# anibali/dsnt-pose2d

Measured on AMD Instinct MI355X. Metric: images/sec (train step, 256x256, 16 joints), higher is better.
Workload: dtype f32; 1 GPU; hg2 + DSNT + JS reg, 256x256 -> 64x64x16, batch 32 per GPU, RMSprop lr 2.5e-4, train step fwd+loss+bwd+optim; global_batch=32, parallelism=dp1, launches_fwd=210

## Files before the change

### dsnt-pose2d_amd/csrc/api.cpp

```cpp
#include "common.h"
#include <string.h>

static thread_local char g_err[512] = "";

int dsnt_set_error(int code, const char* fmt, ...) {
    va_list ap;
    va_start(ap, fmt);
    vsnprintf(g_err, sizeof(g_err), fmt, ap);
    va_end(ap);
    return code;
}

int dsnt_device_id(void) {
    int d = 0;
    if (hipGetDevice(&d) != hipSuccess || d < 0) d = 0;
    return d < DSNT_MAX_DEVICES ? d : DSNT_MAX_DEVICES - 1;
}

int dsnt_device_cus(void) {
    static std::atomic<int> cus[DSNT_MAX_DEVICES];
    const int d = dsnt_device_id();
    int c = cus[d].load(std::memory_order_acquire);
    if (!c) {
        hipDeviceProp_t prop;
        int dev = 0;
        c = (hipGetDevice(&dev) == hipSuccess && hipGetDeviceProperties(&prop, dev) == hipSuccess && prop.multiProcessorCount > 0)
                ? prop.multiProcessorCount : 256;
        cus[d].store(c, std::memory_order_release);
    }
    return c;
}

extern "C" int dsnt_version(void) { return 132; }
extern "C" const char* dsnt_last_error(void) { return g_err; }

#include <vector>
#include <new>

struct dsnt_list {
    struct Entry {
        int kind;
        int lane, src, dst;
        mutable hipEvent_t ev;
        std::function<void(hipStream_t)> fn;
    };
    std::vector<Entry> entries;
    std::vector<size_t> seg_start;
    dsnt_list() { seg_start.push_back(0); }
// ... 78 lines not shown
```

### dsnt-pose2d_amd/csrc/bn.hip

```cpp
#include "common.h"
#include <string.h>
#include "bn_pro.h"
#include "ew_bodies.h"

template <int MODE>
__global__ __launch_bounds__(256) void tile_reduce_kernel(
    const float* __restrict__ a, const float* __restrict__ x, const float* __restrict__ scale,
    const float* __restrict__ shift, const float* __restrict__ mean,
    const float* __restrict__ invstd, int relu, float* __restrict__ partial, long M, int C, int cgs,
    const float* __restrict__ ymask = nullptr, float* __restrict__ dz_out = nullptr) {
    __shared__ float red[256 * 8];
    const int tid = threadIdx.x;
    const int C4 = C >> 2;
    const int rpar = 256 / cgs;
    const int cg_l = tid % cgs, rl = tid / cgs;
    const bool active = rl < rpar;
    const long row0 = (long)blockIdx.x * TILE_ROWS;
    const long row1 = row0 + TILE_ROWS < M ? row0 + TILE_ROWS : M;
    for (int cg0 = blockIdx.y * cgs; cg0 < C4; cg0 += cgs * gridDim.y) {
        const int cg = cg0 + cg_l;
        float4 s1 = make_float4(0.f, 0.f, 0.f, 0.f), s2 = s1;
        if (active && cg < C4) {
            float4 sc, sh, mu, is;
            if (MODE == 1) {
// ... 326 lines not shown
                                long n4) {
    for (long i = (long)blockIdx.x * blockDim.x + threadIdx.x; i < n4; i += (long)gridDim.x * blockDim.x) {
        const float4 g = dy[i], v = y[i];
        dz[i] = make_float4(v.x > 0.f ? g.x : 0.f, v.y > 0.f ? g.y : 0.f, v.z > 0.f ? g.z : 0.f, v.w > 0.f ? g.w : 0.f);
    }
}

extern "C" int dsnt_relu_bwd(const float* dy, const float* y, float* dz, int64_t n, void* stream) {
    DSNT_REQUIRE(dy && y && dz && n > 0 && n % 4 == 0, DSNT_ERR_ARG, "dsnt_relu_bwd: bad argument");
    DSNT_REQUIRE(dsnt_aligned16(dy) && dsnt_aligned16(y) && dsnt_aligned16(dz), DSNT_ERR_ALIGN, "dsnt_relu_bwd: alignment");
    DSNT_LAUNCH(relu_bwd_kernel, dim3(flat_grid(n / 4, 256)), dim3(256), 0, (hipStream_t)stream,
                       (const float4*)dy, (const float4*)y, (float4*)dz, (long)(n / 4));
    DSNT_CHECK_LAUNCH("dsnt_relu_bwd");
}

struct BnApplyVec { float4 sc, sh, mu, is, c0, c1; };
__device__ __forceinline__ float4 bn_apply_one(const float4 g, const float4 xv, const BnApplyVec& v, int relu) {
    float4 dz = g;
    if (relu) {
        if (fmaf(xv.x, v.sc.x, v.sh.x) <= 0.f) dz.x = 0.f;
        if (fmaf(xv.y, v.sc.y, v.sh.y) <= 0.f) dz.y = 0.f;
        if (fmaf(xv.z, v.sc.z, v.sh.z) <= 0.f) dz.z = 0.f;
        if (fmaf(xv.w, v.sc.w, v.sh.w) <= 0.f) dz.w = 0.f;
    }
    float4 o;
    o.x = v.sc.x * (dz.x - v.c0.x - (xv.x - v.mu.x) * v.is.x * v.c1.x);
    o.y = v.sc.y * (dz.y - v.c0.y - (xv.y - v.mu.y) * v.is.y * v.c1.y);
    o.z = v.sc.z * (dz.z - v.c0.z - (xv.z - v.mu.z) * v.is.z * v.c1.z);
    o.w = v.sc.w * (dz.w - v.c0.w - (xv.w - v.mu.w) * v.is.w * v.c1.w);
    return o;
}
struct BnApplyP {
    const float4* da; const float4* x; const float4* scale; const float4* shift; const float4* mean; const float4* invstd;
    const float4* coef; int relu; float4* dx; const float4* base; long n4; int C4; unsigned* amax; BnBwdProP pro;
};
template <bool FIXED>
__global__ void bn_act_bwd_apply_kernel(BnApplyP q) {
    __shared__ double pro_sh[512];
    const float4* __restrict__ da = q.da; const float4* __restrict__ x = q.x; const float4* __restrict__ scale = q.scale;
    const float4* __restrict__ shift = q.shift; const float4* __restrict__ mean = q.mean; const float4* __restrict__ invstd = q.invstd;
    const float4* coef = q.coef; const int relu = q.relu; float4* dx = q.dx; const float4* base = q.base;
    const long n4 = q.n4; const int C4 = q.C4; unsigned* __restrict__ amax = q.amax; const BnBwdProP pro = q.pro;
    const bool accumulate = base != nullptr;
    const int wg = blockIdx.x, nwg = gridDim.x;
    if (pro.partial) {
        bn_pro_backward<256>(pro, pro_sh, wg == 0);
        __syncthreads();
    }
    float am = 0.f;
    const long stride = (long)nwg * 256;
    long i = threadIdx.x < 256 ? (long)wg * 256 + threadIdx.x : n4;
    auto vec = [&](int cg) {
        BnApplyVec v;
        v.sc = scale[cg]; v.sh = shift[cg]; v.mu = mean[cg]; v.is = invstd[cg]; v.c0 = coef[cg]; v.c1 = coef[C4 + cg];
        return v;
    };
    auto amx = [&](const float4 o) { am = fmaxf(fmaxf(fmaxf(fabsf(o.x), fabsf(o.y)), fmaxf(fabsf(o.z), fabsf(o.w))), am); };
    if (FIXED) {
        const BnApplyVec v = vec((int)((i < n4 ? i : 0) % C4));
        for (; i + stride < n4; i += 2 * stride) {
            const float4 g0 = da[i], x0 = x[i], g1 = da[i + stride], x1 = x[i + stride];
            float4 p0 = make_float4(0.f, 0.f, 0.f, 0.f), p1 = p0;
            if (accumulate) { p0 = base[i]; p1 = base[i + stride]; }
            float4 o0 = bn_apply_one(g0, x0, v, relu), o1 = bn_apply_one(g1, x1, v, relu);
            if (accumulate) {
                o0.x += p0.x; o0.y += p0.y; o0.z += p0.z; o0.w += p0.w;
                o1.x += p1.x; o1.y += p1.y; o1.z += p1.z; o1.w += p1.w;
            }
            dx[i] = o0; dx[i + stride] = o1;
            amx(o0); amx(o1);
        }
        if (i < n4) {
            float4 o = bn_apply_one(da[i], x[i], v, relu);
            if (accumulate) { const float4 p = base[i]; o.x += p.x; o.y += p.y; o.z += p.z; o.w += p.w; }
            dx[i] = o;
            amx(o);
        }
    } else {
        for (; i < n4; i += stride) {
            float4 o = bn_apply_one(da[i], x[i], vec((int)(i % C4)), relu);
            if (accumulate) { const float4 p = base[i]; o.x += p.x; o.y += p.y; o.z += p.z; o.w += p.w; }
            dx[i] = o;
            amx(o);
        }
    }
    if (amax) amax_commit(am, amax);
}

static int bn_act_bwd_apply_impl(const float* da, const float* x, const float* scale, const float* shift,
                                 const float* mean, const float* invstd, const float* coef, int relu, float* dx,
                                 int accumulate, int64_t M, int C, float* amax, void* stream, const BnBwdProP* pro, const float* base) {
    DSNT_REQUIRE(da && x && scale && shift && mean && invstd && coef && dx && M > 0 && C > 0,
                 DSNT_ERR_ARG, "dsnt_bn_act_bwd_apply: bad argument");
    DSNT_REQUIRE(C % 4 == 0 && dsnt_aligned16(da) && dsnt_aligned16(x) && dsnt_aligned16(dx) &&
                 dsnt_aligned16(coef) && dsnt_aligned16(base), DSNT_ERR_ALIGN, "dsnt_bn_act_bwd_apply: alignment");
    if (!base && accumulate) base = dx;
    const long n4 = (long)M * C / 4;
    int grid = flat_grid(n4, 256);
    BnBwdProP q;
    memset(&q, 0, sizeof(q));
    if (pro) {
        q = *pro;
        if (grid > 128) grid = 128;
    }
    const BnApplyP ap{(const float4*)da, (const float4*)x, (const float4*)scale, (const float4*)shift, (const float4*)mean,
                      (const float4*)invstd, (const float4*)coef, relu, (float4*)dx, (const float4*)base, n4, C / 4, (unsigned*)amax, q};
    if (((long)grid * 256) % (C / 4) == 0)
        DSNT_LAUNCH(bn_act_bwd_apply_kernel<true>, dim3(grid), dim3(256), 0, stream, ap);
    else
        DSNT_LAUNCH(bn_act_bwd_apply_kernel<false>, dim3(grid), dim3(256), 0, stream, ap);
    DSNT_CHECK_LAUNCH("dsnt_bn_act_bwd_apply");
}

extern "C" int dsnt_bn_act_bwd_apply_amax(const float* da, const float* x, const float* scale,
                                          const float* shift, const float* mean, const float* invstd,
                                          const float* coef, int relu, float* dx, int accumulate,
                                          int64_t M, int C, float* amax, void* stream) {
    return bn_act_bwd_apply_impl(da, x, scale, shift, mean, invstd, coef, relu, dx, accumulate, M, C, amax, stream, nullptr, nullptr);
}

extern "C" int dsnt_bn_act_bwd_apply(const float* da, const float* x, const float* scale,
                                     const float* shift, const float* mean, const float* invstd,
                                     const float* coef, int relu, float* dx, int accumulate,
                                     int64_t M, int C, void* stream) {
    return bn_act_bwd_apply_impl(da, x, scale, shift, mean, invstd, coef, relu, dx, accumulate, M, C, nullptr, stream, nullptr, nullptr);
// ... 19 lines not shown
extern "C" int dsnt_bn_act_bwd_apply_base(const float* da, const float* x, const float* scale, const float* shift,
                                          const float* mean, const float* invstd, const float* coef, int relu,
                                          const float* base, float* dx, int64_t M, int C, float* amax, void* stream) {
    DSNT_REQUIRE(base && base != dx, DSNT_ERR_ARG, "dsnt_bn_act_bwd_apply_base: `base` must be a second tensor");
    return bn_act_bwd_apply_impl(da, x, scale, shift, mean, invstd, coef, relu, dx, 1, M, C, amax, stream, nullptr, base);
}
extern "C" int dsnt_bn_act_bwd_apply_pro_base(const float* da, const float* x, const float* scale, const float* shift,
                                              const float* mean, const float* invstd, const float* partial, int ntiles,
                                              float* dgamma, float* dbeta, int accumulate_params, float* coef, int relu,
                                              const float* base, float* dx, int64_t M, int C, float* amax, void* stream) {
    DSNT_REQUIRE(base && base != dx, DSNT_ERR_ARG, "dsnt_bn_act_bwd_apply_pro_base: `base` must be a second tensor");
    BnBwdProP q;
    if (int e = bn_bwd_pro_fill(q, "dsnt_bn_act_bwd_apply_pro_base", partial, ntiles, dgamma, dbeta, accumulate_params, coef, M, C)) return e;
    return bn_act_bwd_apply_impl(da, x, scale, shift, mean, invstd, coef, relu, dx, 1, M, C, amax, stream, &q, base);
}
```

### dsnt-pose2d_amd/csrc/ew_bodies.h

```cpp
#pragma once
#include "common.h"
#include "bn_pro.h"

#define TILE_ROWS 128
static inline int tile_cgs(long tiles, int C4) { return tiles < 256 && C4 > 16 && C4 % 16 == 0 ? 16 : (C4 < 256 ? C4 : 256); }
static inline unsigned tile_grid_y(long tiles, int C4) { const int c = tile_cgs(tiles, C4); return c == 16 && C4 > 16 ? C4 / 16 : 1; }

struct TileOpP {
    const float* a; const float* b; float* y; unsigned char* idx; float* partial;
    int N, Ho, Wo, C, cgs;
    OutBoundsP tail;
    const float* bn_scale; const float* bn_shift; int bn_relu;
};
template <int OP>
__device__ __forceinline__ void tile_op_stats_body(const TileOpP& q, const int bx, const int by, const int gy, float* red) {
    const float* __restrict__ a = q.a; const float* __restrict__ b = q.b; float* __restrict__ y = q.y;
    unsigned char* __restrict__ idx = q.idx; float* partial = q.partial;
    const int N = q.N, Ho = q.Ho, Wo = q.Wo, C = q.C, cgs = q.cgs;
    const OutBoundsP tail = q.tail;
    const float* __restrict__ bn_scale = q.bn_scale; const float* __restrict__ bn_shift = q.bn_shift; const int bn_relu = q.bn_relu;
    const int tid = threadIdx.x;
    const int C4 = C >> 2;
    const int rpar = 256 / cgs;
    const int cg_l = tid % cgs, rl = tid / cgs;
// ... 110 lines not shown
```

### dsnt-pose2d_amd/csrc/resample.hip

```cpp
#include "common.h"
#include "bn_pro.h"
#include "ew_bodies.h"

__global__ void maxpool2_fwd_kernel(const float4* __restrict__ x, float4* __restrict__ y,
                                    uchar4* __restrict__ idx, int N, int H, int W, int C4) {
    const int Ho = H >> 1, Wo = W >> 1;
    const long total = (long)N * Ho * Wo * C4;
    for (long i = (long)blockIdx.x * blockDim.x + threadIdx.x; i < total;
         i += (long)gridDim.x * blockDim.x) {
        const int cg = (int)(i % C4);
        long t = i / C4;
        const int ow = (int)(t % Wo); t /= Wo;
        const int oh = (int)(t % Ho);
        const int n = (int)(t / Ho);
        const float4* base = x + (((long)n * H + 2 * oh) * W + 2 * ow) * C4 + cg;
        const float4 v0 = base[0], v1 = base[C4], v2 = base[(long)W * C4], v3 = base[(long)W * C4 + C4];
        float4 m = v0;
        uchar4 k = make_uchar4(0, 0, 0, 0);
#define POOL_STEP(V, P)                                  \
        if (V.x > m.x || V.x != V.x) { m.x = V.x; k.x = P; } \
        if (V.y > m.y || V.y != V.y) { m.y = V.y; k.y = P; } \
        if (V.z > m.z || V.z != V.z) { m.z = V.z; k.z = P; } \
        if (V.w > m.w || V.w != V.w) { m.w = V.w; k.w = P; }
        POOL_STEP(v1, 1) POOL_STEP(v2, 2) POOL_STEP(v3, 3)
// ... 72 lines not shown
    DSNT_LAUNCH(maxpool2_bwd_kernel, dim3(flat_grid(total, 256)), dim3(256), 0, stream, q);
    DSNT_CHECK_LAUNCH("dsnt_maxpool2_bwd");
}
extern "C" int dsnt_maxpool2_bwd(const float* dy, const uint8_t* idx, float* dx, int accumulate,
                                 int N, int H, int W, int C, void* stream) {
    return maxpool2_bwd_impl(dy, idx, dx, accumulate, nullptr, N, H, W, C, nullptr, stream);
}
extern "C" int dsnt_maxpool2_bwd_amax(const float* dy, const uint8_t* idx, float* dx, int accumulate,
                                      int N, int H, int W, int C, float* amax, void* stream) {
    return maxpool2_bwd_impl(dy, idx, dx, accumulate, nullptr, N, H, W, C, amax, stream);
}
extern "C" int dsnt_maxpool2_bwd_add(const float* dy, const uint8_t* idx, float* dx, int accumulate, const float* extra,
                                     int N, int H, int W, int C, float* amax, void* stream) {
    DSNT_REQUIRE(extra && extra != dx && dsnt_aligned16(extra), DSNT_ERR_ARG, "dsnt_maxpool2_bwd_add: `extra` must be a second, aligned tensor");
    return maxpool2_bwd_impl(dy, idx, dx, accumulate, extra, N, H, W, C, amax, stream);
}

__global__ void upsample2_add_fwd_kernel(const float4* __restrict__ up, const float4* __restrict__ low,
                                         float4* __restrict__ out, int N, int H, int W, int C4) {
    const long total = (long)N * H * W * C4;
    for (long i = (long)blockIdx.x * blockDim.x + threadIdx.x; i < total;
         i += (long)gridDim.x * blockDim.x) {
        const int cg = (int)(i % C4);
        long t = i / C4;
        const int w = (int)(t % W); t /= W;
        const int h = (int)(t % H);
        const int n = (int)(t / H);
        const float4 a = up[i];
        const float4 b = low[(((long)n * (H >> 1) + (h >> 1)) * (W >> 1) + (w >> 1)) * C4 + cg];
        out[i] = make_float4(a.x + b.x, a.y + b.y, a.z + b.z, a.w + b.w);
// ... 185 lines not shown
```

### dsnt-pose2d_amd/dsnt/_lib.py

```python
import ctypes as C
import os

import torch

_HERE = os.path.dirname(os.path.abspath(__file__))
LIB_PATH = os.environ.get('DSNT_HIP_LIB') or os.path.join(os.path.dirname(_HERE), 'csrc', 'libdsnt_hip.so')

P = C.c_void_p
I = C.c_int
L = C.c_int64
F = C.c_float
D = C.c_double


class ConvGeom(C.Structure):
    _fields_ = [(n, C.c_int) for n in
                ('N', 'H', 'W', 'Cin', 'Ho', 'Wo', 'Cout', 'R', 'S', 'stride', 'pad', 'dil')]


GP = C.POINTER(ConvGeom)


class BnBwdEpilogue(C.Structure):
    _fields_ = [('x', C.c_void_p), ('scale', C.c_void_p), ('shift', C.c_void_p), ('mean', C.c_void_p),
# ... 82 lines not shown
    'dsnt_conv_wgrad_group': [P, I, I, P],
    'dsnt_bn_stats': [P, P, L, I, P],
    'dsnt_bn_finalize': [P, I, L, I, P, P, P, P, F, F, I, P, P, P, P, P],
    'dsnt_bn_act_fwd': [P, P, P, I, P, L, I, P],
    'dsnt_bn_act_bwd_reduce': [P, P, P, P, P, P, I, P, L, I, P],
    'dsnt_bn_bwd_finalize': [P, I, L, I, P, P, I, P, P],
    'dsnt_bn_bwd_finalize_bound': [P, I, L, I, P, P, I, P, P, P, P, P],
    'dsnt_bn_eval_prep': [P, I, P],
    'dsnt_bn_act_bwd_apply': [P, P, P, P, P, P, P, I, P, I, L, I, P],
    'dsnt_bn_act_bwd_apply_amax': [P, P, P, P, P, P, P, I, P, I, L, I, P, P],
    'dsnt_bn_act_bwd_apply_pro': [P, P, P, P, P, P, P, I, P, P, I, P, I, P, I, L, I, P, P],
    'dsnt_stem4_fwd_f16x3': [P, P, L, P, P, P, P, P, GP, TP, P],
    'dsnt_bn_add_act_bwd_reduce': [P, P, P, P, P, I, P, P, L, I, P],
    'dsnt_bn_act_bwd_apply_base': [P, P, P, P, P, P, P, I, P, P, L, I, P, P],
    'dsnt_bn_act_bwd_apply_pro_base': [P, P, P, P, P, P, P, I, P, P, I, P, I, P, P, L, I, P, P],
    'dsnt_conv_fwd_pro': [P, P, P, P, PP, I, P, P, P, GP, TP, P],
    'dsnt_fill_zero': [P, L, P],
    'dsnt_axpy_amax': [P, P, F, I, L, P, P],
    'dsnt_maxpool2_bwd_amax': [P, P, P, I, I, I, I, I, P, P],
    'dsnt_maxpool2_bwd_add': [P, P, P, I, P, I, I, I, I, P, P],
    'dsnt_upsample2_bwd_amax': [P, P, I, I, I, I, I, P, P],
    'dsnt_maxpool2_fwd': [P, P, P, I, I, I, I, P],
    'dsnt_maxpool2_bwd': [P, P, P, I, I, I, I, I, P],
    'dsnt_maxpool2_fwd_stats': [P, P, P, P, I, I, I, I, TP, P],
    'dsnt_upsample2_add_fwd_stats': [P, P, P, P, I, I, I, I, TP, P],
    'dsnt_bn_act_fwd_stats': [P, P, P, I, P, P, L, I, TP, P],
    'dsnt_s2d_input': [P, P, I, I, I, I, TP, P],
    'dsnt_s2d_weights': [P, P, I, I, P],
    'dsnt_s2d_weights_prep': [P, P, P, P, P, I, P],
    'dsnt_maxpool3s2_fwd': [P, P, P, I, I, I, I, P],
# ... 131 lines not shown
```

### dsnt-pose2d_amd/dsnt/engine.py

```python
import os

import torch

from . import _lib, convop
from ._lib import ConvGeom, BnTail
from .bounds import Bounds
from .launchlist import Lanes, LaunchList
from .wgrad_queue import WgradQueue

BN_EPS = 1e-5
BN_MOMENTUM = 0.1


class Act:
    __slots__ = ('buf', 'N', 'H', 'W', 'C', '_grad', 'stats', 'name', 'grad_amax', 'amax_tail', 'fold_ok',
                 'pending_apply', 'uses', 'gives_away', 'is_branch', 'grad_shared', 'pending_add', 'base', 'base_amax')

    def __init__(self, buf, name=''):
        self.buf = buf
        self.N, self.H, self.W, self.C = buf.shape
        self._grad = None
        self.base, self.base_amax = None, None
        self.stats = None
        self.amax_tail = None
# ... 72 lines not shown
        self._keep = []
        self.lib = _lib.load()
        self.nbytes = 0
        self._read_switches()
        lanes = Lanes(self.use_lanes, self.n_lanes)
        self.fwd, self.bwd = (LaunchList(self.lib, lanes, self._keep) for _ in range(2))
        self.bounds = Bounds(self)
        self.wgrads = WgradQueue(self)
        self.lane = 0
        self.cur_bucket = 0
        self._ident = None
        self.acts = []
        self.param_arena = None
        self._planar_src = {}
        self.f16_uses = []

    def _read_switches(self):
        self.use_bf16x6 = os.environ.get('DSNT_MFMA', 'bf16x6') != 'f32'
        self.bf16x6_min_rows = int(os.environ.get('DSNT_BF16X6_MIN_ROWS', '4096'))
        self.use_lanes = os.environ.get('DSNT_LANES', '1') != '0'
        self.side_lanes = (1, 3)
        self.n_lanes = 3 + len(self.side_lanes) - 1
        self.chain_lanes = (0,) + self.side_lanes
        self.wgrad_lane = 2 if (self.use_lanes and os.environ.get('DSNT_WGRAD_LANE', '1') != '0') else None
        self.wgrad_lane_rows = int(os.environ.get('DSNT_X_WGRAD_LANE_ROWS', '16000'))
        self.release_rows = int(os.environ.get('DSNT_X_RELEASE_ROWS', '4096'))
        off = set(os.environ.get('DSNT_OFF', '').replace('+', ',').split(','))
        self.conv3s = 'conv3s' not in off
        self.bwd1 = 'bwd1' not in off
        self.fwd1 = 'fwd1' not in off
        self.fold3 = 'fold3' not in off
        self.fold3_rows = int(os.environ.get('DSNT_X_FOLD3_ROWS', '16384'))
        self.stem4 = 'stem4' not in off
        self.ds_fuse = 'dsfuse' not in off
        self.ds_fuse_rows = int(os.environ.get('DSNT_X_DS_FUSE_ROWS', '65536'))
        self._x = dict(kv.split('=') for kv in os.environ.get('DSNT_X', '').split(',') if '=' in kv)
        self.wgrad_narrow = self._x.get('wgrad_narrow', '1')
        self.share_grads = self._x.get('share_grads', '1') != '0'
        self.defer_res = self._x.get('defer_res', '1') != '0'
        self.flush_points = self._x.get('flush_points', '1') != '0'
        self.prep_split = self._x.get('prep_split', '1') != '0'
        self.defer_reduce = os.environ.get('DSNT_DEFER_REDUCE', '1') != '0'
        self.group_rows = int(os.environ.get('DSNT_X_GROUP_ROWS', '8192')) if self.defer_reduce else 0
        self.fuse_finalize = os.environ.get('DSNT_FUSE_FINALIZE', '1') != '0'
        self.fuse_finalize_max = int(os.environ.get('DSNT_X_FUSE_FINALIZE_MAX', '2048'))
        self.use_f16x3 = self.use_bf16x6 and os.environ.get('DSNT_SPLIT', 'f16x3') == 'f16x3'
        if self.record and not self.training:
            self.use_f16x3 = False
        self.no_relu = bool(os.environ.get('DSNT_DEBUG_NO_RELU'))

# ... 248 lines not shown
        if not finalised:
            acc_p = 1 if bn.uses > 0 else 0
            bn.uses += 1
            if not fused:
                self.b('dsnt_bn_bwd_finalize', part, tiles, x.M, bn.C, bn.ggamma, bn.gbeta, acc_p | (2 if frozen else 0), coef)
        buf, acc, base = self.grad_target_base(x, amax=True)
        if fused:
            coef = self.empty(2 * bn.C)
            if base is not None:
                self.b('dsnt_bn_act_bwd_apply_pro_base', da, x.buf, n.scale, n.shift, n.mean, n.invstd, part, tiles,
                       bn.ggamma, bn.gbeta, acc_p, coef, relu, base, buf, x.M, bn.C, x.grad_amax)
            else:
                self.b('dsnt_bn_act_bwd_apply_pro', da, x.buf, n.scale, n.shift, n.mean, n.invstd, part, tiles,
                       bn.ggamma, bn.gbeta, acc_p, coef, relu, buf, acc, x.M, bn.C, x.grad_amax)
        elif base is not None:
            self.b('dsnt_bn_act_bwd_apply_base', da, x.buf, n.scale, n.shift, n.mean, n.invstd, coef, relu,
                   base, buf, x.M, bn.C, x.grad_amax)
        else:
            self.b_amax('dsnt_bn_act_bwd_apply', da, x.buf, n.scale, n.shift, n.mean, n.invstd, coef, relu,
                        buf, acc, x.M, bn.C, amax=x.grad_amax)

    def conv(self, src, p, res1=None, res2=None, want_stats=False, need_input_grad=True, name=''):
        c = convop.ConvOp(self, src, p, res1, res2, name, need_input_grad)
        c.y = y = self.act(c.x.N, c.g.Ho, c.g.Wo, p.Cout, name)
        c.x.uses += 1
        for r in (res1, res2):
            if r is not None:
                r.uses += 1
                y.gives_away = True
        c.forward(want_stats)
        if self.record:
            c.plan_backward()
            self.on_backward(c.backward)
        return y

# ... 34 lines not shown
        if self.record:
            def backward():
                self._norm_backward(n, y.grad)
            self.on_backward(backward)
        return y

    def maxpool2(self, x, name=''):
        y = self.act(x.N, x.H // 2, x.W // 2, x.C, name)
        x.uses += 1
        idx = self.empty(x.N, x.H // 2, x.W // 2, x.C, dtype=torch.uint8)
        self._f_with_stats('dsnt_maxpool2_fwd', y, (x.buf, y.buf, idx), (x.N, x.H, x.W, x.C))
        if self.record:
            def backward():
                add, x.pending_add = x.pending_add, None
                buf, acc = self.grad_target(x, amax=True, take_add=True)
                if add is not None:
                    assert acc == 1
                    self.b('dsnt_maxpool2_bwd_add', y.grad, idx, buf, acc, add[0], x.N, x.H, x.W, x.C, x.grad_amax)
                else:
                    self.b_amax('dsnt_maxpool2_bwd', y.grad, idx, buf, acc, x.N, x.H, x.W, x.C, amax=x.grad_amax)
            self.on_backward(backward)
        return y

    def maxpool3s2(self, x, name=''):
        Ho, Wo = (x.H - 1) // 2 + 1, (x.W - 1) // 2 + 1
        y = self.act(x.N, Ho, Wo, x.C, name)
        x.uses += 1
        idx = self.empty(x.N, Ho, Wo, x.C, dtype=torch.uint8)
        self.f('dsnt_maxpool3s2_fwd', x.buf, y.buf, idx, x.N, x.H, x.W, x.C)
        if self.record:
            def backward():
# ... 31 lines not shown
        return y

    def upsample2_add(self, up, low, name=''):
        out = self.act(up.N, up.H, up.W, up.C, name)
        up.uses += 1
        low.uses += 1
        out.gives_away = True
        self._f_with_stats('dsnt_upsample2_add_fwd', out, (up.buf, low.buf, out.buf), (up.N, up.H, up.W, up.C))
        if self.record:
            point = self.wgrads.release_point(low.M)

            def backward():
                if point:
                    self.wgrads.pass_release_point()
                buf, acc = self.grad_target(low, amax=True)
                self.b_amax('dsnt_upsample2_bwd', out.grad, buf, acc, up.N, up.H, up.W, up.C, amax=low.grad_amax)
                self.grad_identity(up, out.grad, donate=True, g_amax=out.grad_amax)
            self.on_backward(backward)
        return out

    def to_planar(self, x, C_logical, name='', out=None, gin=None):
        out = self.empty(x.N, C_logical, x.H, x.W) if out is None else out
        x.uses += 1
        if gin is None:
            gin = self.empty(x.N, C_logical, x.H, x.W) if self.record else None
        self.f('dsnt_nhwc_to_nchw', x.buf, out, x.N, C_logical, x.H * x.W, x.C)
        if self.record:
            def backward():
                assert x.grad is None, 'planar output must be the first gradient writer'
                buf, _ = self.grad_target(x)
                self.b('dsnt_nchw_to_nhwc', gin, buf, x.N, C_logical, x.H * x.W, x.C)
# ... 33 lines not shown
```

### dsnt-pose2d_amd/dsnt/launchlist.py

```python
import contextlib
import ctypes as C

import torch

from . import _lib


def check(lib, rc, name):
    if rc != 0:
        raise RuntimeError('%s failed (%d): %s' % (name, rc, lib.dsnt_last_error().decode()))


class Lanes:

    def __init__(self, use, n):
        self.use, self.n = use, n
        self.side = None

    def streams(self):
        main = torch.cuda.current_stream()
        if not self.use:
            return (main, None, None)
        if self.side is None:
            self.side = tuple(torch.cuda.Stream() for _ in range(self.n - 1))
# ... 38 lines not shown
                conv.append(a)
        entry = (fn, tuple(conv), name, lane)
        self._into.append(entry)
        return entry

    @staticmethod
    def sync_entry(src, dst):
        return (None, (src, dst, torch.cuda.Event()), 'sync', 0)

    def sync(self, src, dst):
        self._into.append(self.sync_entry(src, dst))

    def mark(self, k, lane):
        self._into.append((None, k, 'bucket', lane))

    def record(self):
        lib, lanes = self.lib, self.lanes
        h = lib.dsnt_list_create()
        if not h:
            raise RuntimeError('dsnt_list_create failed')
        marks = []
        try:
            for lane in range(1, lanes.n) if lanes.use else ():
                check(lib, lib.dsnt_list_sync(h, 0, lane), 'dsnt_list_sync')
            check(lib, lib.dsnt_list_begin(h), 'dsnt_list_begin')
            try:
                for fn, args, name, lane in self:
                    if fn is not None:
                        check(lib, fn(*args, C.c_void_p(lane)), name)
                    elif name == 'sync':
# ... 61 lines not shown
```

### include/dsnt_hip.h

```cpp
#ifndef DSNT_HIP_H
#define DSNT_HIP_H

#include <stdint.h>

#ifdef __cplusplus
extern "C" {
#endif

typedef enum {
    DSNT_OK = 0,
    DSNT_ERR_SHAPE = 1,
    DSNT_ERR_ALIGN = 2,
    DSNT_ERR_ARG = 3,
    DSNT_ERR_HIP = 4
} dsnt_status;

typedef struct {
    float* amax;
    float* amax_bn; const float* amax_scale; const float* amax_shift; int amax_relu, reserved;
} dsnt_out_bounds;

typedef struct dsnt_bn_prologue {
    const float* partial; int tiles, C;
    int64_t M;
// ... 239 lines not shown
                          int64_t M, int C, void* stream);
int dsnt_bn_act_bwd_apply_amax(const float* da, const float* x, const float* scale, const float* shift,
                               const float* mean, const float* invstd, const float* coef, int relu, float* dx,
                               int accumulate, int64_t M, int C, float* amax, void* stream);
int dsnt_bn_act_bwd_apply_pro(const float* da, const float* x, const float* scale, const float* shift,
                              const float* mean, const float* invstd, const float* partial, int ntiles,
                              float* dgamma, float* dbeta, int accumulate_params, float* coef, int relu,
                              float* dx, int accumulate, int64_t M, int C, float* amax, void* stream);
int dsnt_bn_act_bwd_apply_base(const float* da, const float* x, const float* scale, const float* shift,
                               const float* mean, const float* invstd, const float* coef, int relu,
                               const float* base, float* dx, int64_t M, int C, float* amax, void* stream);
int dsnt_bn_act_bwd_apply_pro_base(const float* da, const float* x, const float* scale, const float* shift,
                                   const float* mean, const float* invstd, const float* partial, int ntiles,
                                   float* dgamma, float* dbeta, int accumulate_params, float* coef, int relu,
                                   const float* base, float* dx, int64_t M, int C, float* amax, void* stream);
int dsnt_fill_zero(float* p, int64_t n, void* stream);
int dsnt_axpy_amax(const float* x, float* y, float a, int accumulate, int64_t n, float* amax, void* stream);
int dsnt_maxpool2_bwd_amax(const float* dy, const uint8_t* idx, float* dx, int accumulate, int N, int H, int W, int C,
                           float* amax, void* stream);
int dsnt_maxpool2_bwd_add(const float* dy, const uint8_t* idx, float* dx, int accumulate, const float* extra,
                          int N, int H, int W, int C, float* amax, void* stream);
int dsnt_upsample2_bwd_amax(const float* dout, float* dlow, int accumulate, int N, int H, int W, int C, float* amax,
                            void* stream);

int dsnt_maxpool2_fwd(const float* x, float* y, uint8_t* idx, int N, int H, int W, int C,
                      void* stream);
int dsnt_maxpool2_bwd(const float* dy, const uint8_t* idx, float* dx, int accumulate,
                      int N, int H, int W, int C, void* stream);

int dsnt_maxpool3s2_fwd(const float* x, float* y, uint8_t* idx, int N, int H, int W, int C, void* stream);
int dsnt_maxpool3s2_bwd(const float* dy, const uint8_t* idx, float* dx, int accumulate, int N, int H, int W,
                        int C, void* stream);
int dsnt_bn_add_act_fwd(const float* x, const float* scale, const float* shift, const float* res, int relu,
                        float* y, int64_t M, int C, void* stream);
int dsnt_relu_bwd(const float* dy, const float* y, float* dz, int64_t n, void* stream);
int dsnt_zero_insert(const float* dy, float* out, int N, int Ho, int Wo, int C, int Hs, int Ws, int stride,
                     void* stream);

// ... 174 lines not shown
```

Before: 2938 images/sec.

## Fold BN backward apply into upsample and maxpool backward kernels

Adds fused kernels that compute the BN+ReLU backward apply and, in the same pass, the 2x upsample backward sum or the maxpool 2x2 backward scatter. The launch-list builder retracts or replaces the previously emitted apply launch when it is the lane's tail and no blocking syncs intervene. This removes one kernel launch and a full write-then-reread of the intermediate gradient per fused pair. It relies on the launch list's tail bookkeeping being correct. The maxpool variant also skips writing the BN output gradient, which is assumed to have no other consumer.

New measurement: 2966 images/sec, median of 6. Within noise of the previous version (+0.9%).

```diff
diff --git a/dsnt-pose2d_amd/csrc/api.cpp b/dsnt-pose2d_amd/csrc/api.cpp
--- a/dsnt-pose2d_amd/csrc/api.cpp
+++ b/dsnt-pose2d_amd/csrc/api.cpp
@@ -31,7 +31,7 @@
     return c;
 }
 
-extern "C" int dsnt_version(void) { return 132; }
+extern "C" int dsnt_version(void) { return 133; }
 extern "C" const char* dsnt_last_error(void) { return g_err; }
 
 #include <vector>
diff --git a/dsnt-pose2d_amd/csrc/bn.hip b/dsnt-pose2d_amd/csrc/bn.hip
--- a/dsnt-pose2d_amd/csrc/bn.hip
+++ b/dsnt-pose2d_amd/csrc/bn.hip
@@ -364,27 +364,12 @@
     DSNT_CHECK_LAUNCH("dsnt_relu_bwd");
 }
 
-struct BnApplyVec { float4 sc, sh, mu, is, c0, c1; };
-__device__ __forceinline__ float4 bn_apply_one(const float4 g, const float4 xv, const BnApplyVec& v, int relu) {
-    float4 dz = g;
-    if (relu) {
-        if (fmaf(xv.x, v.sc.x, v.sh.x) <= 0.f) dz.x = 0.f;
-        if (fmaf(xv.y, v.sc.y, v.sh.y) <= 0.f) dz.y = 0.f;
-        if (fmaf(xv.z, v.sc.z, v.sh.z) <= 0.f) dz.z = 0.f;
-        if (fmaf(xv.w, v.sc.w, v.sh.w) <= 0.f) dz.w = 0.f;
-    }
-    float4 o;
-    o.x = v.sc.x * (dz.x - v.c0.x - (xv.x - v.mu.x) * v.is.x * v.c1.x);
-    o.y = v.sc.y * (dz.y - v.c0.y - (xv.y - v.mu.y) * v.is.y * v.c1.y);
-    o.z = v.sc.z * (dz.z - v.c0.z - (xv.z - v.mu.z) * v.is.z * v.c1.z);
-    o.w = v.sc.w * (dz.w - v.c0.w - (xv.w - v.mu.w) * v.is.w * v.c1.w);
-    return o;
-}
 struct BnApplyP {
     const float4* da; const float4* x; const float4* scale; const float4* shift; const float4* mean; const float4* invstd;
     const float4* coef; int relu; float4* dx; const float4* base; long n4; int C4; unsigned* amax; BnBwdProP pro;
+    float4* dlow; int accumulate_low, H, W; unsigned* amax_low;
 };
-template <bool FIXED>
+template <bool FIXED, bool UP>
 __global__ void bn_act_bwd_apply_kernel(BnApplyP q) {
     __shared__ double pro_sh[512];
     const float4* __restrict__ da = q.da; const float4* __restrict__ x = q.x; const float4* __restrict__ scale = q.scale;
@@ -406,7 +391,45 @@
         return v;
     };
     auto amx = [&](const float4 o) { am = fmaxf(fmaxf(fmaxf(fabsf(o.x), fabsf(o.y)), fmaxf(fabsf(o.z), fabsf(o.w))), am); };
-    if (FIXED) {
+    if (UP) {
+        float4* dlow = q.dlow; const int accumulate_low = q.accumulate_low; const int H = q.H, W = q.W;
+        const int Hl = H >> 1, Wl = W >> 1;
+        const long row = (long)W * C4;
+        float aml = 0.f;
+        BnApplyVec v;
+        if (FIXED) v = vec((int)((i < n4 ? i : 0) % C4));
+        for (; i < n4; i += stride) {
+            const int cg = (int)(i % C4);
+            long t = i / C4;
+            const int w = (int)(t % Wl); t /= Wl;
+            const int h = (int)(t % Hl);
+            const int n = (int)(t / Hl);
+            const long j = (((long)n * H + 2 * h) * W + 2 * w) * C4 + cg;
+            if (!FIXED) v = vec(cg);
+            const float4 g0 = da[j], g1 = da[j + C4], g2 = da[j + row], g3 = da[j + row + C4];
+            const float4 x0 = x[j], x1 = x[j + C4], x2 = x[j + row], x3 = x[j + row + C4];
+            float4 p0 = make_float4(0.f, 0.f, 0.f, 0.f), p1 = p0, p2 = p0, p3 = p0, c = p0;
+            if (accumulate) { p0 = base[j]; p1 = base[j + C4]; p2 = base[j + row]; p3 = base[j + row + C4]; }
+            if (accumulate_low) c = dlow[i];
+            float4 v0 = bn_apply_one(g0, x0, v, relu), v1 = bn_apply_one(g1, x1, v, relu);
+            float4 v2 = bn_apply_one(g2, x2, v, relu), v3 = bn_apply_one(g3, x3, v, relu);
+            if (accumulate) {
+                v0.x += p0.x; v0.y += p0.y; v0.z += p0.z; v0.w += p0.w;
+                v1.x += p1.x; v1.y += p1.y; v1.z += p1.z; v1.w += p1.w;
+                v2.x += p2.x; v2.y += p2.y; v2.z += p2.z; v2.w += p2.w;
+                v3.x += p3.x; v3.y += p3.y; v3.z += p3.z; v3.w += p3.w;
+            }
+            as_stored(v0); as_stored(v1); as_stored(v2); as_stored(v3);
+            dx[j] = v0; dx[j + C4] = v1; dx[j + row] = v2; dx[j + row + C4] = v3;
+            amx(v0); amx(v1); amx(v2); amx(v3);
+            float4 o = make_float4((v0.x + v1.x) + (v2.x + v3.x), (v0.y + v1.y) + (v2.y + v3.y),
+                                   (v0.z + v1.z) + (v2.z + v3.z), (v0.w + v1.w) + (v2.w + v3.w));
+            if (accumulate_low) { o.x += c.x; o.y += c.y; o.z += c.z; o.w += c.w; }
+            dlow[i] = o;
+            aml = fmaxf(fmaxf(fmaxf(fabsf(o.x), fabsf(o.y)), fmaxf(fabsf(o.z), fabsf(o.w))), aml);
+        }
+        if (q.amax_low) amax_commit(aml, q.amax_low, 1);
+    } else if (FIXED) {
         const BnApplyVec v = vec((int)((i < n4 ? i : 0) % C4));
         for (; i + stride < n4; i += 2 * stride) {
             const float4 g0 = da[i], x0 = x[i], g1 = da[i + stride], x1 = x[i + stride];
@@ -437,15 +460,23 @@
     if (amax) amax_commit(am, amax);
 }
 
+struct BnApplyUp { float* dlow; int accumulate; int N, H, W; float* amax; };
 static int bn_act_bwd_apply_impl(const float* da, const float* x, const float* scale, const float* shift,
                                  const float* mean, const float* invstd, const float* coef, int relu, float* dx,
-                                 int accumulate, int64_t M, int C, float* amax, void* stream, const BnBwdProP* pro, const float* base) {
+                                 int accumulate, int64_t M, int C, float* amax, void* stream, const BnBwdProP* pro, const float* base,
+                                 const BnApplyUp* up = nullptr) {
     DSNT_REQUIRE(da && x && scale && shift && mean && invstd && coef && dx && M > 0 && C > 0,
                  DSNT_ERR_ARG, "dsnt_bn_act_bwd_apply: bad argument");
+    if (up) {
+        DSNT_REQUIRE(up->dlow && up->N > 0 && up->H > 0 && up->W > 0, DSNT_ERR_ARG, "dsnt_bn_act_bwd_apply_up: bad argument");
+        DSNT_REQUIRE(up->H % 2 == 0 && up->W % 2 == 0 && (int64_t)up->N * up->H * up->W == M, DSNT_ERR_SHAPE,
+                     "dsnt_bn_act_bwd_apply_up: H and W must be even and N * H * W the M of dx (got %dx%dx%d)", up->N, up->H, up->W);
+    }
     DSNT_REQUIRE(C % 4 == 0 && dsnt_aligned16(da) && dsnt_aligned16(x) && dsnt_aligned16(dx) &&
-                 dsnt_aligned16(coef) && dsnt_aligned16(base), DSNT_ERR_ALIGN, "dsnt_bn_act_bwd_apply: alignment");
+                 dsnt_aligned16(coef) && dsnt_aligned16(base) && (!up || dsnt_aligned16(up->dlow)), DSNT_ERR_ALIGN,
+                 "dsnt_bn_act_bwd_apply: alignment");
     if (!base && accumulate) base = dx;
-    const long n4 = (long)M * C / 4;
+    const long n4 = up ? (long)M / 4 * (C / 4) : (long)M * C / 4;
     int grid = flat_grid(n4, 256);
     BnBwdProP q;
     memset(&q, 0, sizeof(q));
@@ -454,11 +485,17 @@
         if (grid > 128) grid = 128;
     }
     const BnApplyP ap{(const float4*)da, (const float4*)x, (const float4*)scale, (const float4*)shift, (const float4*)mean,
-                      (const float4*)invstd, (const float4*)coef, relu, (float4*)dx, (const float4*)base, n4, C / 4, (unsigned*)amax, q};
-    if (((long)grid * 256) % (C / 4) == 0)
-        DSNT_LAUNCH(bn_act_bwd_apply_kernel<true>, dim3(grid), dim3(256), 0, stream, ap);
+                      (const float4*)invstd, (const float4*)coef, relu, (float4*)dx, (const float4*)base, n4, C / 4, (unsigned*)amax, q,
+                      up ? (float4*)up->dlow : nullptr, up ? up->accumulate : 0, up ? up->H : 0, up ? up->W : 0,
+                      up ? (unsigned*)up->amax : nullptr};
+    const bool fixed = ((long)grid * 256) % (C / 4) == 0;
+    if (up) {
+        if (fixed) DSNT_LAUNCH((bn_act_bwd_apply_kernel<true, true>), dim3(grid), dim3(256), 0, stream, ap);
+        else DSNT_LAUNCH((bn_act_bwd_apply_kernel<false, true>), dim3(grid), dim3(256), 0, stream, ap);
+    } else if (fixed)
+        DSNT_LAUNCH((bn_act_bwd_apply_kernel<true, false>), dim3(grid), dim3(256), 0, stream, ap);
     else
-        DSNT_LAUNCH(bn_act_bwd_apply_kernel<false>, dim3(grid), dim3(256), 0, stream, ap);
+        DSNT_LAUNCH((bn_act_bwd_apply_kernel<false, false>), dim3(grid), dim3(256), 0, stream, ap);
     DSNT_CHECK_LAUNCH("dsnt_bn_act_bwd_apply");
 }
 
@@ -508,3 +545,19 @@
     if (int e = bn_bwd_pro_fill(q, "dsnt_bn_act_bwd_apply_pro_base", partial, ntiles, dgamma, dbeta, accumulate_params, coef, M, C)) return e;
     return bn_act_bwd_apply_impl(da, x, scale, shift, mean, invstd, coef, relu, dx, 1, M, C, amax, stream, &q, base);
 }
+
+extern "C" int dsnt_bn_act_bwd_apply_up(const float* da, const float* x, const float* scale, const float* shift, const float* mean,
+                                        const float* invstd, const float* coef, int relu, float* dx, int accumulate, int64_t M,
+                                        int C, float* amax, float* dlow, int accumulate_low, int N, int H, int W, float* amax_low,
+                                        void* stream) {
+    const BnApplyUp up{dlow, accumulate_low, N, H, W, amax_low};
+    return bn_act_bwd_apply_impl(da, x, scale, shift, mean, invstd, coef, relu, dx, accumulate, M, C, amax, stream, nullptr, nullptr, &up);
+}
+extern "C" int dsnt_bn_act_bwd_apply_base_up(const float* da, const float* x, const float* scale, const float* shift,
+                                             const float* mean, const float* invstd, const float* coef, int relu,
+                                             const float* base, float* dx, int64_t M, int C, float* amax, float* dlow,
+                                             int accumulate_low, int N, int H, int W, float* amax_low, void* stream) {
+    DSNT_REQUIRE(base && base != dx, DSNT_ERR_ARG, "dsnt_bn_act_bwd_apply_base_up: `base` must be a second tensor");
+    const BnApplyUp up{dlow, accumulate_low, N, H, W, amax_low};
+    return bn_act_bwd_apply_impl(da, x, scale, shift, mean, invstd, coef, relu, dx, 1, M, C, amax, stream, nullptr, base, &up);
+}
diff --git a/dsnt-pose2d_amd/csrc/ew_bodies.h b/dsnt-pose2d_amd/csrc/ew_bodies.h
--- a/dsnt-pose2d_amd/csrc/ew_bodies.h
+++ b/dsnt-pose2d_amd/csrc/ew_bodies.h
@@ -5,6 +5,25 @@
 #define TILE_ROWS 128
 static inline int tile_cgs(long tiles, int C4) { return tiles < 256 && C4 > 16 && C4 % 16 == 0 ? 16 : (C4 < 256 ? C4 : 256); }
 static inline unsigned tile_grid_y(long tiles, int C4) { const int c = tile_cgs(tiles, C4); return c == 16 && C4 > 16 ? C4 / 16 : 1; }
+
+struct BnApplyVec { float4 sc, sh, mu, is, c0, c1; };
+__device__ __forceinline__ float4 bn_apply_one(const float4 g, const float4 xv, const BnApplyVec& v, int relu) {
+    float4 dz = g;
+    if (relu) {
+        if (fmaf(xv.x, v.sc.x, v.sh.x) <= 0.f) dz.x = 0.f;
+        if (fmaf(xv.y, v.sc.y, v.sh.y) <= 0.f) dz.y = 0.f;
+        if (fmaf(xv.z, v.sc.z, v.sh.z) <= 0.f) dz.z = 0.f;
+        if (fmaf(xv.w, v.sc.w, v.sh.w) <= 0.f) dz.w = 0.f;
+    }
+    float4 o;
+    o.x = v.sc.x * (dz.x - v.c0.x - (xv.x - v.mu.x) * v.is.x * v.c1.x);
+    o.y = v.sc.y * (dz.y - v.c0.y - (xv.y - v.mu.y) * v.is.y * v.c1.y);
+    o.z = v.sc.z * (dz.z - v.c0.z - (xv.z - v.mu.z) * v.is.z * v.c1.z);
+    o.w = v.sc.w * (dz.w - v.c0.w - (xv.w - v.mu.w) * v.is.w * v.c1.w);
+    return o;
+}
+
+__device__ __forceinline__ void as_stored(float4& o) { asm volatile("" : "+v"(o.x), "+v"(o.y), "+v"(o.z), "+v"(o.w)); }
 
 struct TileOpP {
     const float* a; const float* b; float* y; unsigned char* idx; float* partial;
diff --git a/dsnt-pose2d_amd/csrc/resample.hip b/dsnt-pose2d_amd/csrc/resample.hip
--- a/dsnt-pose2d_amd/csrc/resample.hip
+++ b/dsnt-pose2d_amd/csrc/resample.hip
@@ -110,6 +110,77 @@
                                      int N, int H, int W, int C, float* amax, void* stream) {
     DSNT_REQUIRE(extra && extra != dx && dsnt_aligned16(extra), DSNT_ERR_ARG, "dsnt_maxpool2_bwd_add: `extra` must be a second, aligned tensor");
     return maxpool2_bwd_impl(dy, idx, dx, accumulate, extra, N, H, W, C, amax, stream);
+}
+
+struct PoolBnP {
+    const float4* da; const uchar4* idx; float4* dx; int accumulate; const float4* x; const float4* scale; const float4* shift;
+    const float4* mean; const float4* invstd; const float4* coef; int relu; const float4* base; int N, H, W, C4; unsigned* amax;
+};
+__global__ void maxpool2_bwd_bn_kernel(PoolBnP q) {
+    const float4* __restrict__ da = q.da; const uchar4* __restrict__ idx = q.idx; float4* dx = q.dx; const int accumulate = q.accumulate;
+    const float4* __restrict__ x = q.x; const float4* __restrict__ base = q.base; const int relu = q.relu;
+    const int H = q.H, W = q.W, C4 = q.C4, N = q.N; unsigned* amax = q.amax;
+    const int Ho = H >> 1, Wo = W >> 1;
+    const long total = (long)N * Ho * Wo * C4;
+    const int wg = blockIdx.x, nwg = gridDim.x;
+    const long stride = (long)nwg * 256;
+    auto vec = [&](int cg) {
+        BnApplyVec v;
+        v.sc = q.scale[cg]; v.sh = q.shift[cg]; v.mu = q.mean[cg]; v.is = q.invstd[cg]; v.c0 = q.coef[cg]; v.c1 = q.coef[C4 + cg];
+        return v;
+    };
+    const bool fixed = stride % C4 == 0;
+    long i = (long)wg * 256 + threadIdx.x;
+    BnApplyVec v = vec((int)((i < total ? i : 0) % C4));
+    float am = 0.f;
+    for (; i < total; i += stride) {
+        const int cg = (int)(i % C4);
+        long t = i / C4;
+        const int ow = (int)(t % Wo); t /= Wo;
+        const int oh = (int)(t % Ho);
+        const int n = (int)(t / Ho);
+        if (!fixed) v = vec(cg);
+        const float4 g0 = da[i], xv = x[i];
+        const uchar4 k = idx[i];
+        float4 b = make_float4(0.f, 0.f, 0.f, 0.f);
+        if (base) b = base[i];
+        float4* win = dx + (((long)n * H + 2 * oh) * W + 2 * ow) * C4 + cg;
+        float4 c[4];
+        if (accumulate) {
+#pragma unroll
+            for (int p = 0; p < 4; ++p) c[p] = win[(p >> 1) * (long)W * C4 + (p & 1) * C4];
+        }
+        float4 g = bn_apply_one(g0, xv, v, relu);
+        if (base) { g.x += b.x; g.y += b.y; g.z += b.z; g.w += b.w; }
+        as_stored(g);
+#pragma unroll
+        for (int p = 0; p < 4; ++p) {
+            float4* d = win + (p >> 1) * (long)W * C4 + (p & 1) * C4;
+            float4 o = make_float4(k.x == p ? g.x : 0.f, k.y == p ? g.y : 0.f, k.z == p ? g.z : 0.f,
+                                   k.w == p ? g.w : 0.f);
+            if (accumulate) { o.x += c[p].x; o.y += c[p].y; o.z += c[p].z; o.w += c[p].w; }
+            *d = o;
+            am = fmaxf(fmaxf(fmaxf(fabsf(o.x), fabsf(o.y)), fmaxf(fabsf(o.z), fabsf(o.w))), am);
+        }
+    }
+    if (amax) amax_commit(am, amax);
+}
+
+extern "C" int dsnt_maxpool2_bwd_bn(const float* da, const uint8_t* idx, float* dx, int accumulate, const float* x,
+                                    const float* scale, const float* shift, const float* mean, const float* invstd,
+                                    const float* coef, int relu, const float* base, int N, int H, int W, int C, float* amax,
+                                    void* stream) {
+    DSNT_REQUIRE(da && idx && dx && x && scale && shift && mean && invstd && coef && N > 0 && H > 0 && W > 0 && C > 0, DSNT_ERR_ARG,
+                 "dsnt_maxpool2_bwd_bn: bad argument");
+    DSNT_REQUIRE(H % 2 == 0 && W % 2 == 0, DSNT_ERR_SHAPE, "dsnt_maxpool2_bwd_bn: H and W must be even");
+    DSNT_REQUIRE(C % 4 == 0 && dsnt_aligned16(da) && dsnt_aligned16(dx) && dsnt_aligned16(x) && dsnt_aligned16(coef) &&
+                 dsnt_aligned16(base) && (((uintptr_t)idx) & 3) == 0, DSNT_ERR_ALIGN, "dsnt_maxpool2_bwd_bn: alignment");
+    const long total = (long)N * (H / 2) * (W / 2) * (C / 4);
+    const PoolBnP q{(const float4*)da, (const uchar4*)idx, (float4*)dx, accumulate, (const float4*)x, (const float4*)scale,
+                    (const float4*)shift, (const float4*)mean, (const float4*)invstd, (const float4*)coef, relu, (const float4*)base,
+                    N, H, W, C / 4, (unsigned*)amax};
+    DSNT_LAUNCH(maxpool2_bwd_bn_kernel, dim3(flat_grid(total, 256)), dim3(256), 0, stream, q);
+    DSNT_CHECK_LAUNCH("dsnt_maxpool2_bwd_bn");
 }
 
 __global__ void upsample2_add_fwd_kernel(const float4* __restrict__ up, const float4* __restrict__ low,
diff --git a/dsnt-pose2d_amd/dsnt/_lib.py b/dsnt-pose2d_amd/dsnt/_lib.py
--- a/dsnt-pose2d_amd/dsnt/_lib.py
+++ b/dsnt-pose2d_amd/dsnt/_lib.py
@@ -120,6 +120,9 @@
     'dsnt_bn_add_act_bwd_reduce': [P, P, P, P, P, I, P, P, L, I, P],
     'dsnt_bn_act_bwd_apply_base': [P, P, P, P, P, P, P, I, P, P, L, I, P, P],
     'dsnt_bn_act_bwd_apply_pro_base': [P, P, P, P, P, P, P, I, P, P, I, P, I, P, P, L, I, P, P],
+    'dsnt_bn_act_bwd_apply_up': [P, P, P, P, P, P, P, I, P, I, L, I, P, P, I, I, I, I, P, P],
+    'dsnt_bn_act_bwd_apply_base_up': [P, P, P, P, P, P, P, I, P, P, L, I, P, P, I, I, I, I, P, P],
+    'dsnt_maxpool2_bwd_bn': [P, P, P, I, P, P, P, P, P, P, I, P, I, I, I, I, P, P],
     'dsnt_conv_fwd_pro': [P, P, P, P, PP, I, P, P, P, GP, TP, P],
     'dsnt_fill_zero': [P, L, P],
     'dsnt_axpy_amax': [P, P, F, I, L, P, P],
diff --git a/dsnt-pose2d_amd/dsnt/engine.py b/dsnt-pose2d_amd/dsnt/engine.py
--- a/dsnt-pose2d_amd/dsnt/engine.py
+++ b/dsnt-pose2d_amd/dsnt/engine.py
@@ -110,6 +110,7 @@
         self.param_arena = None
         self._planar_src = {}
         self.f16_uses = []
+        self._last_apply = {}
 
     def _read_switches(self):
         self.use_bf16x6 = os.environ.get('DSNT_MFMA', 'bf16x6') != 'f32'
@@ -130,6 +131,8 @@
         self.stem4 = 'stem4' not in off
         self.ds_fuse = 'dsfuse' not in off
         self.ds_fuse_rows = int(os.environ.get('DSNT_X_DS_FUSE_ROWS', '65536'))
+        self.upfold = 'upfold' not in off
+        self.poolfold = 'poolfold' not in off
         self._x = dict(kv.split('=') for kv in os.environ.get('DSNT_X', '').split(',') if '=' in kv)
         self.wgrad_narrow = self._x.get('wgrad_narrow', '1')
         self.share_grads = self._x.get('share_grads', '1') != '0'
@@ -408,11 +411,25 @@
                 self.b('dsnt_bn_act_bwd_apply_pro', da, x.buf, n.scale, n.shift, n.mean, n.invstd, part, tiles,
                        bn.ggamma, bn.gbeta, acc_p, coef, relu, buf, acc, x.M, bn.C, x.grad_amax)
         elif base is not None:
-            self.b('dsnt_bn_act_bwd_apply_base', da, x.buf, n.scale, n.shift, n.mean, n.invstd, coef, relu,
-                   base, buf, x.M, bn.C, x.grad_amax)
+            self._emit_apply('dsnt_bn_act_bwd_apply_base', (da, x.buf, n.scale, n.shift, n.mean, n.invstd, coef, relu,
+                                                            base, buf, x.M, bn.C), x.grad_amax, buf)
         else:
-            self.b_amax('dsnt_bn_act_bwd_apply', da, x.buf, n.scale, n.shift, n.mean, n.invstd, coef, relu,
-                        buf, acc, x.M, bn.C, amax=x.grad_amax)
+            self._emit_apply('dsnt_bn_act_bwd_apply', (da, x.buf, n.scale, n.shift, n.mean, n.invstd, coef, relu,
+                                                       buf, acc, x.M, bn.C), x.grad_amax, buf)
+
+    def _emit_apply(self, name, args, amax, buf):
+        nb = self.bwd.nbytes
+        e = self.b(name, *args, amax) if name.endswith('_base') else self.b_amax(name, *args, amax=amax)
+        self._last_apply[self.lane] = (e, self.bwd.nbytes - nb, name, args, amax, buf)
+
+    def _apply_tail(self, grad, name, blocked):
+        rec = self._last_apply.get(self.lane)
+        if rec is None or grad is None or rec[5].data_ptr() != grad.data_ptr() or rec[2] not in name:
+            return None
+        t = self.bwd.tail(rec[0], self.lane)
+        if t is None or any(blocked(src, dst) for src, dst in t[1]):
+            return None
+        return t[0], rec
 
     def conv(self, src, p, res1=None, res2=None, want_stats=False, need_input_grad=True, name=''):
         c = convop.ConvOp(self, src, p, res1, res2, name, need_input_grad)
@@ -477,7 +494,14 @@
             def backward():
                 add, x.pending_add = x.pending_add, None
                 buf, acc = self.grad_target(x, amax=True, take_add=True)
-                if add is not None:
+                tail = self._apply_tail(y.grad, ('dsnt_bn_act_bwd_apply',), lambda src, dst: src == self.lane) \
+                    if (self.poolfold and add is None) else None
+                if tail is not None:
+                    i, (_, nb, _, a, _, _) = tail
+                    self.bwd.retract(i, nb)
+                    self.b('dsnt_maxpool2_bwd_bn', a[0], idx, buf, acc, *a[1:8], a[8] if a[9] else None,
+                           x.N, x.H, x.W, x.C, x.grad_amax)
+                elif add is not None:
                     assert acc == 1
                     self.b('dsnt_maxpool2_bwd_add', y.grad, idx, buf, acc, add[0], x.N, x.H, x.W, x.C, x.grad_amax)
                 else:
@@ -539,7 +563,14 @@
                 if point:
                     self.wgrads.pass_release_point()
                 buf, acc = self.grad_target(low, amax=True)
-                self.b_amax('dsnt_upsample2_bwd', out.grad, buf, acc, up.N, up.H, up.W, up.C, amax=low.grad_amax)
+                tail = self._apply_tail(out.grad, ('dsnt_bn_act_bwd_apply', 'dsnt_bn_act_bwd_apply_base'),
+                                        lambda src, dst: dst == self.lane) if self.upfold else None
+                if tail is not None:
+                    i, (_, nb, name, a, amax, _) = tail
+                    self.bwd.replace(i, nb, self.lane, name + '_up', *a, amax, buf, acc, up.N, up.H, up.W, low.grad_amax)
+                    del self._last_apply[self.lane]
+                else:
+                    self.b_amax('dsnt_upsample2_bwd', out.grad, buf, acc, up.N, up.H, up.W, up.C, amax=low.grad_amax)
                 self.grad_identity(up, out.grad, donate=True, g_amax=out.grad_amax)
             self.on_backward(backward)
         return out
diff --git a/dsnt-pose2d_amd/dsnt/launchlist.py b/dsnt-pose2d_amd/dsnt/launchlist.py
--- a/dsnt-pose2d_amd/dsnt/launchlist.py
+++ b/dsnt-pose2d_amd/dsnt/launchlist.py
@@ -76,6 +76,32 @@
     def mark(self, k, lane):
         self._into.append((None, k, 'bucket', lane))
 
+    def tail(self, entry, lane):
+        syncs = []
+        for i in range(len(self) - 1, -1, -1):
+            e = self[i]
+            if e is entry:
+                return i, syncs
+            if e[0] is not None:
+                if e[3] == lane:
+                    return None
+            elif e[2] == 'sync':
+                syncs.append(e[1][:2])
+            else:
+                return None
+        return None
+
+    def retract(self, i, nb):
+        self.count(self[i][2], -nb)
+        del self[i]
+
+    def replace(self, i, nb, lane, name, *args):
+        self.count(self[i][2], -nb)
+        with self.into([]) as one:
+            self.emit(lane, name, *args)
+        self[i] = one[0]
+        return one[0]
+
     def record(self):
         lib, lanes = self.lib, self.lanes
         h = lib.dsnt_list_create()
diff --git a/include/dsnt_hip.h b/include/dsnt_hip.h
--- a/include/dsnt_hip.h
+++ b/include/dsnt_hip.h
@@ -277,6 +277,13 @@
                                    const float* mean, const float* invstd, const float* partial, int ntiles,
                                    float* dgamma, float* dbeta, int accumulate_params, float* coef, int relu,
                                    const float* base, float* dx, int64_t M, int C, float* amax, void* stream);
+int dsnt_bn_act_bwd_apply_up(const float* da, const float* x, const float* scale, const float* shift, const float* mean,
+                             const float* invstd, const float* coef, int relu, float* dx, int accumulate, int64_t M, int C,
+                             float* amax, float* dlow, int accumulate_low, int N, int H, int W, float* amax_low, void* stream);
+int dsnt_bn_act_bwd_apply_base_up(const float* da, const float* x, const float* scale, const float* shift, const float* mean,
+                                  const float* invstd, const float* coef, int relu, const float* base, float* dx, int64_t M,
+                                  int C, float* amax, float* dlow, int accumulate_low, int N, int H, int W, float* amax_low,
+                                  void* stream);
 int dsnt_fill_zero(float* p, int64_t n, void* stream);
 int dsnt_axpy_amax(const float* x, float* y, float a, int accumulate, int64_t n, float* amax, void* stream);
 int dsnt_maxpool2_bwd_amax(const float* dy, const uint8_t* idx, float* dx, int accumulate, int N, int H, int W, int C,
@@ -285,6 +292,9 @@
                           int N, int H, int W, int C, float* amax, void* stream);
 int dsnt_upsample2_bwd_amax(const float* dout, float* dlow, int accumulate, int N, int H, int W, int C, float* amax,
                             void* stream);
+int dsnt_maxpool2_bwd_bn(const float* da, const uint8_t* idx, float* dx, int accumulate, const float* x, const float* scale,
+                         const float* shift, const float* mean, const float* invstd, const float* coef, int relu,
+                         const float* base, int N, int H, int W, int C, float* amax, void* stream);
 
 int dsnt_maxpool2_fwd(const float* x, float* y, uint8_t* idx, int N, int H, int W, int C,
                       void* stream);
```
